# michaelriedl/2048-ppo-agent

Measured on AMD Instinct MI355X. Metric: env-steps/sec at N parallel boards (full PPO loop: rollout with policy in the loop + GAE + update), higher is better.
Workload: dtype u8 boards / bf16 policy; 1 GPU; 65536 parallel boards per GPU, Transformer policy bf16 (3.96 M params), full PPO iteration (BASELINE.json configs[2]; configs[3] when n_gpus=8); boards_per_gpu=65536, global_boards=65536, train_batch=2048, update_epochs=5, max_samples_per_epoch=300000, max_samples_per_epoch_is=global (each rank draws its 1/N share), as the reference's single subset, max_samples_per_epoch_per_rank=300000, rollout_mode=episodes (reference lock-step semantics), rng_mode=partitionable, parallelism=env-shard x1 + 1 grad all-reduce/minibatch

## Files before the change

2048-ppo-agent_amd/csrc/g2048_linear.hip:

```cpp
#include <hip/hip_runtime.h>
#include <stdint.h>

#include "../../include/g2048.h"
#include "g2048_colsum_final.h"
#include "g2048_host.h"
#include "g2048_mfma.h"

namespace {

using namespace g2048_mfma;
using namespace g2048_host;

enum { EPI_NONE = 0, EPI_RELU_DROPOUT = 1, EPI_MASK_COLSUM = 2 };
struct Epi {
    float inv_keep;
    uint32_t thr16, s0, s1;
    const uint64_t *seed_state;
    int64_t row_elems;
    uint2 *bits;
    float *partial;
    int N;
    uint32_t hi_term;
};

constexpr int TOK = 128, NS = 128, KC = 128, THREADS = 256;
constexpr int CHUNK_BYTES = NS * KC * 2;
constexpr int NBUF = 2;

__device__ __forceinline__ void dma_chunk(char *dst, const __bf16 *w_slice, int64_t ldw, int kc, int w, int lane) {
    const char *base = reinterpret_cast<const char *>(w_slice) + (size_t)kc * KC * 2;
    for (int t = 0; t < NS / 16; ++t) {
        const int row = 4 * (4 * t + w) + (lane >> 4);
        const int q = (lane & 15) ^ (row & 15);
        const char *g = base + (size_t)row * ldw * 2 + q * 16;
        __builtin_amdgcn_global_load_lds((const __attribute__((address_space(1))) void *)g,
                                         (__attribute__((address_space(3))) void *)(dst + (4 * t + w) * 1024), 16, 0, 0);
    }
}

template <bool HAS_BIAS, int EPI>
__device__ __forceinline__ void store_tile(f32x16 acc[4], const float *__restrict__ bias, __bf16 *yrow, int n0, int h, bool valid,
                                           const Epi &E, int64_t tok, uint2 *bits_slot, uint2 bits_in, float *colacc) {
    uint32_t obits[2] = {0u, 0u};
    const uint32_t pair0 = (uint32_t)(((uint64_t)tok * (uint64_t)E.row_elems + (uint64_t)(n0 + 4 * h)) >> 1);
    for (int j = 0; j < 4; ++j) {
        if (HAS_BIAS)
            for (int g = 0; g < 4; ++g) {
                const float4 bv = *reinterpret_cast<const float4 *>(bias + n0 + 32 * j + 8 * g + 4 * h);
                acc[j][4 * g + 0] += bv.x; acc[j][4 * g + 1] += bv.y; acc[j][4 * g + 2] += bv.z; acc[j][4 * g + 3] += bv.w;
            }
        if (EPI == EPI_RELU_DROPOUT) {
            for (int i = 0; i < 16; i += 2) {
                float a = fmaxf(acc[j][i], 0.f), b = fmaxf(acc[j][i + 1], 0.f);
                if (E.thr16) {
                    uint32_t x = (pair0 + (uint32_t)(16 * j + ((i & 3) >> 1) + 4 * (i >> 2))) * HASH_MUL + E.hi_term;
                    G2048_HASH_FIN(x);
                    a = (x & 0xFFFFu) >= E.thr16 ? a * E.inv_keep : 0.f;
                    b = (x >> 16) >= E.thr16 ? b * E.inv_keep : 0.f;
                }
                acc[j][i] = a; acc[j][i + 1] = b;
            }
        }
        if (EPI == EPI_MASK_COLSUM) {
            const uint32_t w = j < 2 ? bits_in.x : bits_in.y;
            for (int i = 0; i < 16; ++i) acc[j][i] = ((w >> (16 * (j & 1) + i)) & 1u) ? acc[j][i] * E.inv_keep : 0.f;
        }
        for (int m = 0; m < 2; ++m) {
            uint32_t ax = pack2(acc[j][8 * m + 0], acc[j][8 * m + 1]), ay = pack2(acc[j][8 * m + 2], acc[j][8 * m + 3]);
            uint32_t bx = pack2(acc[j][8 * m + 4], acc[j][8 * m + 5]), by = pack2(acc[j][8 * m + 6], acc[j][8 * m + 7]);
            if (EPI == EPI_RELU_DROPOUT) {
                const uint32_t pk[4] = {ax, ay, bx, by};
                for (int q = 0; q < 4; ++q) {
                    const uint32_t nz = ((pk[q] & 0x7FFFu) ? 1u : 0u) | ((pk[q] & 0x7FFF0000u) ? 2u : 0u);
                    obits[j >> 1] |= nz << (16 * (j & 1) + 8 * m + 2 * q);
                }
            }
            const auto sx = __builtin_amdgcn_permlane32_swap(ax, bx, false, false);
            const auto sy = __builtin_amdgcn_permlane32_swap(ay, by, false, false);
            uint32_t o[4] = {sx[0], sy[0], sx[1], sy[1]};
            if (EPI == EPI_MASK_COLSUM) {
                for (int q = 0; q < 4; ++q) {
                    if (!valid) o[q] = 0u;
                    colacc[8 * (2 * j + m) + 2 * q] += __uint_as_float(o[q] << 16);
                    colacc[8 * (2 * j + m) + 2 * q + 1] += __uint_as_float(o[q] & 0xFFFF0000u);
                }
            }
            if (valid) *reinterpret_cast<uint4 *>(yrow + 32 * j + 16 * m) = make_uint4(o[0], o[1], o[2], o[3]);
        }
    }
    if (EPI == EPI_RELU_DROPOUT && bits_slot) *bits_slot = make_uint2(obits[0], obits[1]);
}

template <bool HAS_BIAS>
__global__ void __launch_bounds__(THREADS, 2)
k_linear(const __bf16 *__restrict__ x, int64_t ldx, const __bf16 *__restrict__ wgt, int64_t ldw, const float *__restrict__ bias,
         __bf16 *__restrict__ y, int64_t ldy, int64_t T, int K) {
    extern __shared__ __attribute__((aligned(16))) char smem[];
    const int tid = threadIdx.x, lane = tid & 63, w = tid >> 6, r = lane & 31, h = lane >> 5;
    const int64_t tok0 = (int64_t)blockIdx.x * TOK + 32 * w;
    const int n0 = blockIdx.y * NS;
    const __bf16 *w_slice = wgt + (size_t)n0 * ldw;
    const int n_chunks = K / KC;

    int64_t tok = tok0 + r;
    const bool valid = tok < T;
    if (!valid) tok = T - 1;
    const uint4 *xrow = reinterpret_cast<const uint4 *>(x + tok * ldx) + h;

    uint4 bq[8];
    for (int ks = 0; ks < 8; ++ks) bq[ks] = xrow[2 * ks];
    dma_chunk(smem, w_slice, ldw, 0, w, lane);
    if (n_chunks > 1) dma_chunk(smem + CHUNK_BYTES, w_slice, ldw, 1, w, lane);

    f32x16 acc[4];
    for (int j = 0; j < 4; ++j)
        for (int i = 0; i < 16; ++i) acc[j][i] = 0.f;

    int aoff[8];
    for (int ks = 0; ks < 8; ++ks) aoff[ks] = r * 256 + (((2 * ks + h) ^ (r & 15)) * 16);

    for (int c = 0; c < n_chunks; ++c) {
        if (c + 1 < n_chunks) asm volatile("s_waitcnt vmcnt(8)" ::: "memory");
        else asm volatile("s_waitcnt vmcnt(0)" ::: "memory");
        __syncthreads();
        const char *tile = smem + (c % NBUF) * CHUNK_BYTES;
        bf16x8 b[8];
        for (int ks = 0; ks < 8; ++ks) b[ks] = *reinterpret_cast<const bf16x8 *>(&bq[ks]);
        if (c + 1 < n_chunks)
            for (int ks = 0; ks < 8; ++ks) bq[ks] = xrow[2 * (8 * (c + 1) + ks)];
        for (int ks = 0; ks < 8; ++ks)
            for (int j = 0; j < 4; ++j) {
                const bf16x8 a = *reinterpret_cast<const bf16x8 *>(tile + aoff[ks] + j * 32 * 256);
                acc[j] = __builtin_amdgcn_mfma_f32_32x32x16_bf16(a, b[ks], acc[j], 0, 0, 0);
            }
        __syncthreads();
        if (c + NBUF < n_chunks) dma_chunk(smem + (c % NBUF) * CHUNK_BYTES, w_slice, ldw, c + NBUF, w, lane);
    }
    store_tile<HAS_BIAS, EPI_NONE>(acc, bias, y + (tok0 + r) * ldy + n0 + 8 * h, n0, h, valid, Epi{}, 0, nullptr, make_uint2(0u, 0u), nullptr);
}


constexpr int TOKW = 64;
template <int K, int NF>
struct XTileDma {
    static constexpr int CPR = K / 8, RPI = 64 / CPR, N_INST = TOKW / RPI;
    static constexpr int NVAR = 16 / RPI / NF > 0 ? 16 / RPI / NF : 1;
    static_assert(N_INST % NF == 0, "every wave issues the same number of fetch instructions");
    uint32_t voff[NVAR];
    int sub, p;
    __device__ __forceinline__ void init(int64_t ldx, int lane, int f) {
        sub = lane / CPR, p = lane % CPR;
        for (int v = 0; v < NVAR; ++v)
            voff[v] = (uint32_t)(sub * ldx * 2) + 16u * (uint32_t)(p ^ ((RPI * (NF * v + f) + sub) & 15));
    }
    __device__ __forceinline__ void full(char *dst, const __bf16 *x, int64_t ldx, int64_t tok0, int f) const {
        const char *base = reinterpret_cast<const char *>(x + tok0 * ldx);
#pragma unroll
        for (int j = 0; j < N_INST / NF; ++j) {
            const int n = NF * j + f;
            dma_async16(base + (int64_t)n * RPI * ldx * 2, voff[j % NVAR], dst + n * 1024);
        }
    }
    __device__ __forceinline__ void clamped(char *dst, const __bf16 *x, int64_t ldx, int64_t tok0, int64_t T, int f) const {
        for (int j = 0; j < N_INST / NF; ++j) {
            const int n = NF * j + f;
            const int row = n * RPI + sub;
            int64_t tok = tok0 + row;
            if (tok >= T) tok = T - 1;
            dma_async<16>(reinterpret_cast<const char *>(x + tok * ldx) + (p ^ (row & 15)) * 16, dst + n * 1024);
        }
    }
};

#ifdef G2048_WS_STAMPS
constexpr int WS_PHASES = 8;
__device__ unsigned long long g_ws_stamps[2][WS_PHASES];
struct WsStampSite {
    __device__ __forceinline__ static bool on(int lane, int w) { return lane == 0 && w < 2 && blockIdx.y == 0 && blockIdx.x % 16 == 0; }
    __device__ __forceinline__ static unsigned long long *table(int w) { return g_ws_stamps[w == 0 ? 0 : 1]; }
};
#define WS_STAMP(k) stamps.mark(k)
#else
#define WS_STAMP(k)
#endif

template <bool HAS_BIAS, int EPI, int KS, int WAVES>
__global__ void __launch_bounds__(64 * WAVES, 1)
k_linear_ws(const __bf16 *__restrict__ x, int64_t ldx, const __bf16 *__restrict__ wgt, int64_t ldw, const float *__restrict__ bias,
            __bf16 *__restrict__ y, int64_t ldy, int64_t T, Epi E) {
    constexpr int THREADS = 64 * WAVES, NSW = 32 * WAVES;
    constexpr int CPR_Y = NSW / 8;
    constexpr int K = 16 * KS;
    extern __shared__ __attribute__((aligned(16))) char smem[];
    const int tid = threadIdx.x, lane = tid & 63, r = lane & 31, h = lane >> 5;
    const int w = __builtin_amdgcn_readfirstlane(tid >> 6);
    const int n0 = blockIdx.y * NSW;
    constexpr int row_bytes = K * 2, xbytes = TOKW * row_bytes, sbytes = TOKW * 2 * NSW;

    bf16x8 wf[KS];
    {
        const __bf16 *wrow = wgt + (size_t)(n0 + 32 * w + r) * ldw + 8 * h;
#pragma unroll
        for (int ks = 0; ks < KS; ++ks) wf[ks] = *reinterpret_cast<const bf16x8 *>(wrow + 16 * ks);
    }
    constexpr int NB = 2;
    char *const stage = smem + NB * xbytes;
    float *const bias_l = reinterpret_cast<float *>(smem + NB * xbytes + sbytes);
    uint32_t *const bits_l = reinterpret_cast<uint32_t *>(smem + NB * xbytes + sbytes + NSW * 4);
    for (int i = tid; i < NSW; i += THREADS) bias_l[i] = HAS_BIAS ? bias[n0 + i] : 0.f;
    if (EPI == EPI_RELU_DROPOUT) {
        mix_seed_state(E.seed_state, E.s0, E.s1);
        E.hi_term = E.s0 ^ (E.s1 * HASH_MUL_HI);
    }
    const int slices = gridDim.y;
    float colacc[EPI == EPI_MASK_COLSUM ? 16 : 1];
    for (int q = 0; q < (EPI == EPI_MASK_COLSUM ? 16 : 1); ++q) colacc[q] = 0.f;
    const int64_t n_tiles64 = (T + TOKW - 1) / TOKW;
    auto bits_ptr = [&](int64_t tile) -> uint32_t * {
        return reinterpret_cast<uint32_t *>(E.bits) + (tile * slices + blockIdx.y) * THREADS;
    };
    XTileDma<K, WAVES> dma;
    dma.init(ldx, lane, w);
    auto fetch = [&](int64_t tile, int buf) {
        if ((tile + 1) * TOKW <= T) dma.full(smem + buf * xbytes, x, ldx, tile * TOKW, w);
        else dma.clamped(smem + buf * xbytes, x, ldx, tile * TOKW, T, w);
        if (EPI == EPI_MASK_COLSUM) {
            const uint32_t *g = bits_ptr(tile) + lane;
            dma_async<4>(g + 64 * w, bits_l + buf * THREADS + 64 * w);
        }
    };
    if ((int64_t)blockIdx.x < n_tiles64) fetch(blockIdx.x, 0);
    asm volatile("s_waitcnt vmcnt(0)" ::: "memory");
#ifdef G2048_WS_STAMPS
    Stamps<WS_PHASES, WsStampSite> stamps;
    stamps.start();
#endif
    int buf = 0;
    for (int64_t tile = blockIdx.x; tile < n_tiles64; tile += gridDim.x, buf ^= 1) {
        const int64_t tok0 = tile * TOKW;
        const char *const xb = smem + buf * xbytes;
        lds_barrier_asm();
        WS_STAMP(1);
        if (tile + gridDim.x < n_tiles64) fetch(tile + gridDim.x, buf ^ 1);
        WS_STAMP(2);
        const uint32_t bits_in = EPI == EPI_MASK_COLSUM ? bits_l[buf * THREADS + tid] : 0u;
        f32x16 acc[2];
        for (int g = 0; g < 4; ++g) {
            const float4 bv = *reinterpret_cast<const float4 *>(bias_l + 32 * w + 8 * g + 4 * h);
            for (int b = 0; b < 2; ++b) {
                acc[b][4 * g + 0] = bv.x; acc[b][4 * g + 1] = bv.y; acc[b][4 * g + 2] = bv.z; acc[b][4 * g + 3] = bv.w;
            }
        }
        const int nw = n0 + 32 * w;
        uint32_t obits = 0u;
        auto keep_pair = [&](int pi, uint32_t pair0) -> uint32_t {
            const int i = 2 * pi;
            uint32_t xh = (pair0 + (uint32_t)(((i & 3) >> 1) + 4 * (i >> 2))) * HASH_MUL + E.hi_term;
            G2048_HASH_FIN(xh);
            return ((xh & 0xFFFFu) >= E.thr16 ? 1u : 0u) | ((xh >> 16) >= E.thr16 ? 2u : 0u);
        };
        auto drop_pair = [&](int b, int pi, uint32_t keep) {
            const int i = 2 * pi;
            const float a = fmaxf(acc[b][i], 0.f), c = fmaxf(acc[b][i + 1], 0.f);
            acc[b][i] = (keep & 1u) ? a * E.inv_keep : 0.f;
            acc[b][i + 1] = (keep & 2u) ? c * E.inv_keep : 0.f;
        };
        auto finish_g = [&](int b, int g, bool valid) {
            if (EPI == EPI_MASK_COLSUM) {
                const uint32_t wbits = bits_in >> (16 * b + 4 * g);
#pragma unroll
                for (int j = 0; j < 4; ++j) acc[b][4 * g + j] = ((wbits >> j) & 1u) ? acc[b][4 * g + j] * E.inv_keep : 0.f;
            }
            const uint32_t lo = pack2(acc[b][4 * g + 0], acc[b][4 * g + 1]), hi = pack2(acc[b][4 * g + 2], acc[b][4 * g + 3]);
            if (EPI == EPI_RELU_DROPOUT) {
                const uint32_t nz = ((lo & 0x7FFFu) ? 1u : 0u) | ((lo & 0x7FFF0000u) ? 2u : 0u) | ((hi & 0x7FFFu) ? 4u : 0u) |
                                    ((hi & 0x7FFF0000u) ? 8u : 0u);
                obits |= nz << (16 * b + 4 * g);
            }
            if (EPI == EPI_MASK_COLSUM) {
                colacc[4 * g + 0] += valid ? __uint_as_float(lo << 16) : 0.f;
                colacc[4 * g + 1] += valid ? __uint_as_float(lo & 0xFFFF0000u) : 0.f;
                colacc[4 * g + 2] += valid ? __uint_as_float(hi << 16) : 0.f;
                colacc[4 * g + 3] += valid ? __uint_as_float(hi & 0xFFFF0000u) : 0.f;
            }
            const int trow = 32 * b + r, c = 4 * w + g;
            *reinterpret_cast<uint2 *>(stage + trow * (2 * NSW) + ((c ^ (trow & (CPR_Y - 1))) * 16) + 8 * h) = make_uint2(lo, hi);
        };
        const bool valid0 = tok0 + r < T, valid1 = tok0 + 32 + r < T;
        uint32_t pair0[2];
        for (int b = 0; b < 2; ++b)
            pair0[b] = (uint32_t)(((uint64_t)((b ? valid1 : valid0) ? tok0 + 32 * b + r : T - 1) * (uint64_t)E.row_elems + (uint64_t)(nw + 4 * h)) >> 1);
        {
            constexpr int PRE = 8, N = 2 * KS;
            bf16x8 q[PRE];
            auto frag = [&](int s) {
                const int b = s / KS, ks = s % KS;
                return *reinterpret_cast<const bf16x8 *>(xb + (32 * b + r) * row_bytes + (((2 * ks + h) ^ (r & 15)) * 16));
            };
#pragma unroll
            for (int s = 0; s < PRE; ++s) q[s] = frag(s);
#pragma unroll
            for (int s = 0; s < N; ++s) {
                __builtin_amdgcn_sched_barrier(0);
                const int b = s / KS, ks = s % KS;
                acc[b] = __builtin_amdgcn_mfma_f32_32x32x16_bf16(wf[ks], q[s % PRE], acc[b], 0, 0, 0);
                if (s + PRE < N) q[s % PRE] = frag(s + PRE);
                constexpr int SPG = KS / 4;
                const int g = ks / SPG, t = ks % SPG;
                if (b == 1) {
                    if (EPI == EPI_RELU_DROPOUT) {
                        if (SPG >= 4) {
                            if (t == 0) drop_pair(0, 2 * g, keep_pair(2 * g, pair0[0]));
                            if (t == 2) drop_pair(0, 2 * g + 1, keep_pair(2 * g + 1, pair0[0]));
                        } else if (t == 0) {
                            drop_pair(0, 2 * g, keep_pair(2 * g, pair0[0]));
                            drop_pair(0, 2 * g + 1, keep_pair(2 * g + 1, pair0[0]));
                        }
                    }
                    if (t == SPG - 1) finish_g(0, g, valid0);
                }
            }
            __builtin_amdgcn_sched_barrier(0);
        }
        WS_STAMP(3);
#pragma unroll
        for (int g = 0; g < 4; ++g) {
            if (EPI == EPI_RELU_DROPOUT) {
                drop_pair(1, 2 * g, keep_pair(2 * g, pair0[1]));
                drop_pair(1, 2 * g + 1, keep_pair(2 * g + 1, pair0[1]));
            }
            finish_g(1, g, valid1);
        }
        if (EPI == EPI_RELU_DROPOUT && E.bits) bits_ptr(tile)[tid] = obits;
        WS_STAMP(5);
        asm volatile("s_waitcnt vmcnt(0)" ::: "memory");
        WS_STAMP(0);
        lds_barrier_asm();
        WS_STAMP(6);
        {
            constexpr int PIECES = TOKW * CPR_Y, STORERS = THREADS, ROUNDS = PIECES / STORERS;
            static_assert(PIECES % STORERS == 0, "every lane moves the same number of 16-byte pieces");
            const int e0 = tid;
            uint4 v[ROUNDS];
#pragma unroll
            for (int i = 0; i < ROUNDS; ++i) {
                const int e = e0 + STORERS * i;
                v[i] = *reinterpret_cast<const uint4 *>(stage + (e / CPR_Y) * (2 * NSW) + (e % CPR_Y) * 16);
            }
#pragma unroll
            for (int i = 0; i < ROUNDS; ++i) {
                const int e = e0 + STORERS * i;
                const int trow = e / CPR_Y, p = e % CPR_Y, c = p ^ (trow & (CPR_Y - 1));
                if (tok0 + trow < T) *reinterpret_cast<uint4 *>(y + (tok0 + trow) * ldy + n0 + 8 * c) = v[i];
            }
        }
        WS_STAMP(7);
    }
#ifdef G2048_WS_STAMPS
    stamps.flush(lane, w);
#endif
    if (EPI == EPI_MASK_COLSUM) {
        for (int q = 0; q < 16; ++q) {
            float v = colacc[q];
            for (int m = 16; m >= 1; m >>= 1) v += __shfl_xor(v, m);
            if (r == 0) E.partial[(int64_t)blockIdx.x * E.N + n0 + 32 * w + rowof(q, h)] = v;
        }
    }
}

}

namespace {

inline int ws_waves(int N) { return N % 256 == 0 ? 8 : 4; }
inline int64_t ws_groups(int64_t T, int N) {
    const int waves = ws_waves(N);
    const int64_t n_tiles = (T + TOKW - 1) / TOKW;
    int64_t groups = 256 / (N / (32 * waves));
    if (groups < 1) groups = 1;
    if (groups >= 8) groups -= groups % 8;
    return groups > n_tiles ? n_tiles : groups;
}

inline bool operands_ok(const void *x, int64_t ldx, const void *weight, int64_t ldw, const void *y, int64_t ldy, int64_t T, int K,
                        int N, const void *bias) {
    return x && weight && y && T > 0 && K >= KC && K % KC == 0 && N >= NS && N % NS == 0 && ldx >= K && ldw >= K && ldy >= N &&
           !(ldx & 7) && !(ldw & 7) && !(ldy & 7) && aligned16(x, weight, y, bias);
}

template <bool HAS_BIAS, int EPI, int KS, int WAVES>
int launch_ws(const __bf16 *x, int64_t ldx, const __bf16 *w, int64_t ldw, const float *bias, __bf16 *y, int64_t ldy, int64_t T, int N,
              const Epi &E, int64_t groups, hipStream_t stream) {
    const void *fn = reinterpret_cast<const void *>(k_linear_ws<HAS_BIAS, EPI, KS, WAVES>);
    const int lds = 2 * TOKW * 16 * KS * 2 + TOKW * 2 * 32 * WAVES + 32 * WAVES * 4 + 2 * 64 * WAVES * 4;
    if (const int rc = allow_dynamic_lds(fn, lds)) return rc;
    hipLaunchKernelGGL((k_linear_ws<HAS_BIAS, EPI, KS, WAVES>), dim3((unsigned)groups, (unsigned)(N / (32 * WAVES))), dim3(64 * WAVES), lds,
                       stream, x, ldx, w, ldw, bias, y, ldy, T, E);
    return launch_status();
}
template <bool HAS_BIAS, int EPI>
int launch_stationary(const __bf16 *x, int64_t ldx, const __bf16 *w, int64_t ldw, const float *bias, __bf16 *y, int64_t ldy, int64_t T,
                      int K, int N, const Epi &E, int *groups_out, hipStream_t stream) {
    if (K != 256 && K != 128) return G2048_EINVAL;
    const int64_t groups = ws_groups(T, N);
    if (groups_out) *groups_out = (int)groups;
    const bool wide = ws_waves(N) == 8;
    if (K == 256)
        return wide ? launch_ws<HAS_BIAS, EPI, 16, 8>(x, ldx, w, ldw, bias, y, ldy, T, N, E, groups, stream)
                    : launch_ws<HAS_BIAS, EPI, 16, 4>(x, ldx, w, ldw, bias, y, ldy, T, N, E, groups, stream);
    return wide ? launch_ws<HAS_BIAS, EPI, 8, 8>(x, ldx, w, ldw, bias, y, ldy, T, N, E, groups, stream)
                : launch_ws<HAS_BIAS, EPI, 8, 4>(x, ldx, w, ldw, bias, y, ldy, T, N, E, groups, stream);
}

}

extern "C" int g2048_linear_bf16(const void *x, int64_t ldx, const void *weight, int64_t ldw, const float *bias, void *y,
                                 int64_t ldy, int64_t T, int K, int N, void *stream) {
    if (!operands_ok(x, ldx, weight, ldw, y, ldy, T, K, N, bias)) return G2048_EINVAL;
    const __bf16 *xp = (const __bf16 *)x, *wp = (const __bf16 *)weight;
    __bf16 *yp = (__bf16 *)y;
    if (K <= NBUF * KC)
        return bias ? launch_stationary<true, EPI_NONE>(xp, ldx, wp, ldw, bias, yp, ldy, T, K, N, Epi{}, nullptr, (hipStream_t)stream)
                    : launch_stationary<false, EPI_NONE>(xp, ldx, wp, ldw, bias, yp, ldy, T, K, N, Epi{}, nullptr, (hipStream_t)stream);
    const void *fn = bias ? reinterpret_cast<const void *>(k_linear<true>) : reinterpret_cast<const void *>(k_linear<false>);
    if (const int rc = allow_dynamic_lds(fn, NBUF * CHUNK_BYTES)) return rc;
    const dim3 grid((unsigned)((T + TOK - 1) / TOK), (unsigned)(N / NS));
    if (bias)
        hipLaunchKernelGGL(k_linear<true>, grid, dim3(THREADS), NBUF * CHUNK_BYTES, (hipStream_t)stream, xp, ldx, wp, ldw, bias, yp, ldy, T, K);
    else
        hipLaunchKernelGGL(k_linear<false>, grid, dim3(THREADS), NBUF * CHUNK_BYTES, (hipStream_t)stream, xp, ldx, wp, ldw, bias, yp, ldy, T,
                           K);
    return launch_status();
}

extern "C" int64_t g2048_ffn_mask_bytes(int64_t T, int N) {
    return (T <= 0 || N < NS || N % NS) ? 0 : ((T + TOK - 1) / TOK) * (N / NS) * THREADS * (int64_t)sizeof(uint2);
}

extern "C" int g2048_linear_relu_dropout_bf16(const void *x, int64_t ldx, const void *weight, int64_t ldw, const float *bias, void *y,
                                              int64_t ldy, int64_t T, int K, int N, float p_drop, uint64_t seed,
                                              const uint64_t *seed_state, void *mask_bits, void *stream) {
    if (!operands_ok(x, ldx, weight, ldw, y, ldy, T, K, N, bias) || !bias || K > NBUF * KC || !(p_drop >= 0.f && p_drop < 1.f))
        return G2048_EINVAL;
    Epi E{};
    E.inv_keep = 1.0f / (1.0f - p_drop);
    E.thr16 = (uint32_t)(p_drop * 65536.0f + 0.5f);
    E.s0 = (uint32_t)seed; E.s1 = (uint32_t)(seed >> 32);
    E.seed_state = p_drop > 0.f ? seed_state : nullptr;
    E.row_elems = N;
    E.bits = (uint2 *)mask_bits;
    if ((uintptr_t)mask_bits & 7) return G2048_EINVAL;
    return launch_stationary<true, EPI_RELU_DROPOUT>((const __bf16 *)x, ldx, (const __bf16 *)weight, ldw, bias, (__bf16 *)y, ldy, T, K, N,
                                                     E, nullptr, (hipStream_t)stream);
}

extern "C" int64_t g2048_linear_mask_bwd_workspace_floats(int64_t T, int N) {
    return (T <= 0 || N < NS || N % NS) ? 0 : (int64_t)512 * N;
}

extern "C" int64_t g2048_linear_mask_bwd_partial_rows(int64_t T, int N) {
    if (T <= 0 || N < NS || N % NS) return 0;
    return ws_groups(T, N);
}

extern "C" int g2048_linear_mask_bwd_bf16(const void *dy, int64_t lddy, const void *weight_t, int64_t ldw, const void *mask_bits,
                                          void *dz, int64_t lddz, float *dbias, float *workspace, int64_t T, int K, int N,
                                          float p_drop, void *stream) {
    if (!operands_ok(dy, lddy, weight_t, ldw, dz, lddz, T, K, N, nullptr) || K > NBUF * KC || !mask_bits ||
        ((uintptr_t)mask_bits & 7) || !workspace || !aligned16(workspace) || !(p_drop >= 0.f && p_drop < 1.f))
        return G2048_EINVAL;
    Epi E{};
    E.inv_keep = 1.0f / (1.0f - p_drop);
    E.bits = (uint2 *)const_cast<void *>(mask_bits);
    E.partial = workspace;
    E.N = N;
    int groups = 0;
    const int rc = launch_stationary<false, EPI_MASK_COLSUM>((const __bf16 *)dy, lddy, (const __bf16 *)weight_t, ldw, nullptr, (__bf16 *)dz,
                                                             lddz, T, K, N, E, &groups, (hipStream_t)stream);
    if (rc || !dbias) return rc;
    hipLaunchKernelGGL(k_colsum_final, dim3((unsigned)((N + CF_COLS - 1) / CF_COLS)), dim3(CF_COLS * CF_SLICES), 0, (hipStream_t)stream,
                       workspace, groups, N, dbias);
    return launch_status();
}

#ifdef G2048_WS_STAMPS
extern "C" int g2048_debug_ws_stamps(unsigned long long *out , int reset) {
    if (hipMemcpyFromSymbol(out, HIP_SYMBOL(g_ws_stamps), sizeof(g_ws_stamps)) != hipSuccess) return -1;
    if (reset) {
        static const unsigned long long zero[2][WS_PHASES] = {};
        if (hipMemcpyToSymbol(HIP_SYMBOL(g_ws_stamps), zero, sizeof(zero)) != hipSuccess) return -1;
    }
    return 0;
}
#endif
```

include/g2048.h:

```cpp
#ifndef G2048_H
#define G2048_H

#include <stdint.h>

#ifdef __cplusplus
extern "C" {
#endif

#define G2048_ABI_VERSION 4
#define G2048_EINVAL (-1)
#define G2048_RNG_LEGACY 0
#define G2048_RNG_PARTITIONABLE 1
#define G2048_POLICY_DRUL 0
#define G2048_POLICY_RANDOM 1
#define G2048_MAX_FUSED_STEPS 128

int g2048_abi_version(void);


int g2048_split(uint32_t key0, uint32_t key1, uint32_t *out_keys, int64_t n, int rng_mode, void *stream);

int g2048_chain_keys(uint32_t *key , uint32_t *subs , int64_t n, int rng_mode);


int g2048_init(const uint32_t *keys, uint8_t *boards, uint8_t *masks, uint8_t *done, int64_t B,
               int rng_mode, void *stream);

int g2048_step(uint8_t *boards, uint8_t *masks, uint8_t *done, const int32_t *actions,
               const uint32_t *keys, float *rewards, int64_t B, int rng_mode, void *stream);

int g2048_observe(const uint8_t *boards, uint8_t *obs, int64_t B, void *stream);


int g2048_act_drul(const uint8_t *masks, int32_t *actions, int64_t B, void *stream);
int g2048_act_random(const uint32_t *keys, const uint8_t *masks, int32_t *actions, float *log_probs,
                     int64_t B, int rng_mode, void *stream);
int g2048_act_logits(const uint32_t *keys, const float *logits, const uint8_t *masks, int use_mask,
                     int sample, int32_t *actions, float *log_probs, int64_t B, int rng_mode, void *stream);


int g2048_reset_fused(uint32_t sub0, uint32_t sub1, uint8_t *boards, uint8_t *masks, uint8_t *done,
                      int32_t *ep_len, int64_t B, int64_t B_total, int64_t env0, int rng_mode, void *stream);

int g2048_rollout_fused(const uint32_t *step_subs , int n_steps, int64_t t0, uint8_t *boards,
                        uint8_t *masks, uint8_t *done, int32_t *ep_len, uint8_t *tr_boards,
                        uint8_t *tr_meta, float *tr_rewards, float *tr_logp, int64_t B, int64_t B_total,
                        int64_t env0, int policy, int fill_frozen, int rng_mode, uint32_t *live_count,
                        void *stream);

int g2048_policy_step(uint32_t act_sub0, uint32_t act_sub1, uint32_t step_sub0, uint32_t step_sub1,
                      const float *logits, const float *values, int use_mask, int sample, int64_t t,
                      uint8_t *boards, uint8_t *masks, uint8_t *done, int32_t *ep_len, uint8_t *tr_boards,
                      uint8_t *tr_meta, float *tr_rewards, float *tr_logp, float *tr_values, int64_t B,
                      int64_t B_total, int64_t env0, int fill_frozen, int rng_mode, uint32_t *live_count,
                      void *stream);

int g2048_policy_step_autoreset(uint32_t act_sub0, uint32_t act_sub1, uint32_t step_sub0, uint32_t step_sub1,
                                const float *logits, const float *values, int use_mask, int sample, int64_t t,
                                uint8_t *boards, uint8_t *masks, int32_t *ep_len, uint8_t *tr_boards, uint8_t *tr_meta,
                                float *tr_rewards, float *tr_logp, float *tr_values, int64_t B, int64_t B_total,
                                int64_t env0, int rng_mode, void *stream);
int g2048_reset_key(uint32_t step_sub0, uint32_t step_sub1, uint32_t *out );


int g2048_gae_tb(const float *tr_rewards, const float *tr_values, const int32_t *ep_len, float *tr_adv,
                 float *tr_ret, int64_t T, int64_t B, double gamma, double lam, void *stream);

int g2048_gae_tb_boot(const float *tr_rewards, const float *tr_values, const uint8_t *tr_meta, const float *last_values,
                      float *tr_adv, float *tr_ret, int64_t T, int64_t B, double gamma, double lam, void *stream);

int g2048_gae_flat(const float *rewards, const float *values, const uint8_t *terms, float *adv, float *ret,
                   int64_t N, double gamma, double lam, void *stream);

int g2048_compact(const uint8_t *tr_boards, const uint8_t *tr_meta, const float *tr_rewards, const float *tr_logp,
                  const float *tr_values, const float *tr_adv, const float *tr_ret, const int32_t *ep_len,
                  const int64_t *offsets, uint8_t *out_boards, uint8_t *out_actions, uint8_t *out_masks, float *out_rewards,
                  float *out_logp, float *out_values, float *out_adv, float *out_ret, uint8_t *out_terms, int64_t T,
                  int64_t B, void *stream);


int64_t g2048_policy_encoder_workspace_bytes(int64_t B);
int g2048_policy_encoder(const uint8_t *boards, const float *embed_table, const float *cls_token,
                         const void *weights_bf16, const float *params_f32, int n_layers, float *features,
                         int64_t B, void *workspace, void *stream);

int g2048_policy_encoder_mean(const uint8_t *boards, const float *embed_table, const float *cls_token,
                              const void *weights_bf16, const float *params_f32, int n_layers, float *features,
                              int64_t B, void *stream);

#define G2048_F32SPLIT_BIAS 0
#define G2048_F32SPLIT_BIAS_RELU 1
#define G2048_F32SPLIT_ADD_LN 2
#define G2048_F32SPLIT_ADD 3

int g2048_f32split_pack(const float *w, int N, int K, float scale, void *packed, void *stream);

int g2048_f32split_gemm(const float *x, int64_t ldx, const void *w_packed, const float *bias, float *y, int64_t ldy,
                        const float *resid, const float *gamma, const float *beta, float *h, int64_t T, int K, int N,
                        int epilogue, float sx, float sw, float eps, void *stream);

int g2048_attn_fwd_f32(const float *qkv, float *o, int64_t B, int H, float scale, void *stream);

int g2048_embed_ln_f32(const uint8_t *boards, const float *table, const float *cls, const float *gamma, const float *beta, float eps,
                       float *x0, float *h, int64_t B, void *stream);


int g2048_lookahead_expand(const uint8_t *boards, int64_t B, uint8_t *after, float *reward, int32_t *nchild, void *stream);

int g2048_lookahead_children(const uint8_t *after, const int32_t *nchild, const int32_t *offset, int64_t B, int64_t N,
                             uint8_t *children, uint8_t *terminal, void *stream);

int g2048_lookahead_reduce(const float *reward, const int32_t *nchild, const int32_t *offset, const float *values,
                           const uint8_t *terminal, double gamma, int64_t B, int64_t N, float *q, void *stream);


int g2048_lookahead_dedup(const uint8_t *after, const int32_t *nchild, const int32_t *group_start, int64_t G, int64_t P, int32_t *rep,
                          int32_t *nuniq, void *stream);

int g2048_lookahead_backup(const float *reward, const int32_t *nchild, const int32_t *rep, const float *e, int64_t N1, float *v1,
                           void *stream);


int g2048_sym_canon(const uint8_t *boards, const uint8_t *actions, const uint8_t *masks, int64_t B, uint8_t *out_boards,
                    uint8_t *out_actions, uint8_t *out_masks, uint8_t *frame, void *stream);

int g2048_sym_logits(const float *logits, const uint8_t *frame, int64_t B, float *out, void *stream);


int g2048_sym_views(const uint8_t *boards, int64_t B, uint8_t *views, void *stream);

int g2048_sym_fold(const float *logits, const float *values, int64_t B, float *out_logits, float *out_values, void *stream);


int g2048_mc_playout(const uint32_t *step_subs , int n_steps, int64_t t0, const uint8_t *roots, int64_t B, int R,
                     int64_t lane0, int64_t n_total, int policy, double gamma, uint8_t *lane_boards, uint8_t *lane_masks,
                     uint8_t *lane_done, float *lane_ret, float *lane_disc, int rng_mode, uint32_t *live_count, void *stream);

int g2048_mc_reduce(const float *lane_ret, const float *lane_disc, const uint8_t *lane_done, const float *leaf_values, int64_t B,
                    int R, float *q, void *stream);


int g2048_ntuple_values(const uint8_t *boards, int64_t n, const int32_t *weights, const uint8_t *tuple_cells , int m, int L,
                        int frac_bits, float *values, void *stream);

int g2048_ntuple_scores(const uint8_t *boards, int64_t B, const int32_t *weights, const uint8_t *tuple_cells , int m, int L,
                        int frac_bits, float *scores, float *values, void *stream);

int g2048_ntuple_td_accumulate(const uint8_t *prev_after, const uint8_t *flag, const float *target, int64_t B,
                               const int32_t *weights, const uint8_t *tuple_cells , int m, int L, int frac_bits, double alpha,
                               int64_t *acc, int32_t *cnt, float *td_error, void *stream);

int g2048_ntuple_td_apply(const uint8_t *prev_after, const uint8_t *flag, int64_t B, const uint8_t *tuple_cells , int m, int L,
                          int32_t *weights, int64_t *acc, int32_t *cnt, void *stream);

int g2048_ntuple_link(const uint8_t *tr_boards_row, const uint8_t *tr_meta_row, int64_t B, uint8_t *prev_after, uint8_t *flag,
                      void *stream);


int64_t g2048_ntuple_expectimax_workspace_floats(int64_t B, int plies);

int g2048_ntuple_expectimax(const uint8_t *boards, int64_t B, const int32_t *weights, const uint8_t *tuple_cells , int m,
                            int L, int frac_bits, int plies, double gamma, float *workspace, float *scores, float *values,
                            void *stream);


int g2048_ntuple_tc_accumulate(const uint8_t *prev_after, const uint8_t *flag, const float *target, int64_t B,
                               const int32_t *weights, const uint8_t *tuple_cells , int m, int L, int frac_bits, double alpha,
                               int64_t *acc, int64_t *abs_acc, int32_t *cnt, float *td_error, void *stream);

int g2048_ntuple_tc_apply(const uint8_t *prev_after, const uint8_t *flag, int64_t B, const uint8_t *tuple_cells , int m, int L,
                          int32_t *weights, int64_t *acc, int64_t *abs_acc, int32_t *cnt, int32_t *coh_e, int32_t *coh_a,
                          void *stream);

int g2048_ntuple_staged_values(const uint8_t *boards, int64_t n, const int32_t *weights, const uint8_t *tuple_cells , int m,
                               int L, const uint8_t *stage_tiles , int n_stages, int frac_bits, float *values, void *stream);
int g2048_ntuple_staged_scores(const uint8_t *boards, int64_t B, const int32_t *weights, const uint8_t *tuple_cells , int m,
                               int L, const uint8_t *stage_tiles , int n_stages, int frac_bits, float *scores, float *values,
                               void *stream);
int g2048_ntuple_staged_expectimax(const uint8_t *boards, int64_t B, const int32_t *weights, const uint8_t *tuple_cells ,
                                   int m, int L, const uint8_t *stage_tiles , int n_stages, int frac_bits, int plies,
                                   double gamma, float *workspace, float *scores, float *values, void *stream);
int g2048_ntuple_staged_td_accumulate(const uint8_t *prev_after, const uint8_t *flag, const float *target, int64_t B,
                                      const int32_t *weights, const uint8_t *tuple_cells , int m, int L,
                                      const uint8_t *stage_tiles , int n_stages, int frac_bits, double alpha, int64_t *acc,
                                      int32_t *cnt, float *td_error, void *stream);
int g2048_ntuple_staged_td_apply(const uint8_t *prev_after, const uint8_t *flag, int64_t B, const uint8_t *tuple_cells , int m,
                                 int L, const uint8_t *stage_tiles , int n_stages, int32_t *weights, int64_t *acc,
                                 int32_t *cnt, void *stream);
int g2048_ntuple_staged_tc_accumulate(const uint8_t *prev_after, const uint8_t *flag, const float *target, int64_t B,
                                      const int32_t *weights, const uint8_t *tuple_cells , int m, int L,
                                      const uint8_t *stage_tiles , int n_stages, int frac_bits, double alpha, int64_t *acc,
                                      int64_t *abs_acc, int32_t *cnt, float *td_error, void *stream);
int g2048_ntuple_staged_tc_apply(const uint8_t *prev_after, const uint8_t *flag, int64_t B, const uint8_t *tuple_cells , int m,
                                 int L, const uint8_t *stage_tiles , int n_stages, int32_t *weights, int64_t *acc,
                                 int64_t *abs_acc, int32_t *cnt, int32_t *coh_e, int32_t *coh_a, void *stream);


int g2048_attn_fwd(const void *q, const void *k, const void *v, void *o, float *lse, int64_t B, int H, int Sq,
                   int64_t q_sb, int64_t q_ss, int64_t k_sb, int64_t k_ss, int64_t v_sb, int64_t v_ss, float scale,
                   float p_drop, uint64_t seed, const uint64_t *seed_state, void *stream);
int g2048_attn_bwd(const void *q, const void *k, const void *v, const void *dout, const float *lse, void *dq, void *dk,
                   void *dv, int64_t B, int H, int Sq, int64_t q_sb, int64_t q_ss, int64_t k_sb, int64_t k_ss,
                   int64_t v_sb, int64_t v_ss, float scale, float p_drop, uint64_t seed, const uint64_t *seed_state,
                   void *stream);


int g2048_add_ln_fwd(const float *x, int64_t x_row_stride, const void *a, const float *gamma, const float *beta,
                     float *x_new, void *h, float *mean, float *rstd, int64_t T, float eps, float p_drop,
                     uint64_t seed, const uint64_t *seed_state, void *stream);
int64_t g2048_add_ln_bwd_workspace_floats(int64_t T);
int g2048_add_ln_bwd(const float *x_norm, int64_t x_row_stride, const float *g_x, const void *g_h, const float *mean,
                     const float *rstd, const float *gamma, float *dx, void *da, float *dparams, float *workspace,
                     int64_t T, float p_drop, uint64_t seed, const uint64_t *seed_state, int g_x_period, void *stream);


int g2048_linear_add_ln_fwd(const void *u, int64_t ldu, const void *w_packed, const float *bias, int K, const float *x,
                            int64_t x_row_stride, const float *gamma, const float *beta, float *x_new, void *h, float *mean,
                            float *rstd, int64_t T, float eps, float p_drop, uint64_t seed, const uint64_t *seed_state, void *stream);
int64_t g2048_linear_add_ln_bwd_partial_rows(int64_t T);
int g2048_linear_add_ln_bwd(const void *dy, int64_t lddy, const void *wt_packed, int64_t wt_tile_stride, int K, const float *x_norm,
                            int64_t x_row_stride, const float *g_x, int g_x_period, const void *g_h_extra, int extra_period,
                            const float *mean, const float *rstd, const float *gamma, float *dx, void *da, float *partial, int64_t T,
                            float p_drop, uint64_t seed, const uint64_t *seed_state, void *stream);


int g2048_mlp_embed_fwd(const uint8_t *boards, const void *wt, const float *bias, void *y, void *onehot, int64_t M, void *stream);

#define G2048_GEMM_MAX_JOBS 8
typedef struct {
    const void *x[2]; int64_t ldx[2];
    const void *w[2]; int64_t ldw[2];
    int32_t k[2];
    const float *bias;
    const void *act; int64_t ldact;
    void *y; int64_t ldy;
    int32_t N, relu;
} g2048_gemm_job;
int g2048_gemm_jobs(const g2048_gemm_job *jobs, int n_jobs, int64_t M, void *stream);

int g2048_mlp_out_fwd(const void *h2, const void *w3, float *logits, float *values, int64_t M, void *stream);
int64_t g2048_mlp_out_bwd_partial_rows(int64_t M);
int g2048_mlp_out_bwd(const float *dlogits, const float *dvalues, const void *h2, const void *w3, void *dh2, float *partial, int64_t M,
                      void *stream);


#define G2048_COLSUM_MAX_GROUPS 512
int64_t g2048_colsum_workspace_floats(int64_t T, int N);
int64_t g2048_colsum_partial_rows(int64_t T, int N);
int g2048_colsum(const void *x, int is_bf16, int64_t row_stride, int64_t T, int N, float *workspace, float *out,
                 void *stream);


#define G2048_PPO_LOSS_MAX_BATCH 1048576
int g2048_ppo_loss(const void *logits, int logits_bf16, const void *values, int values_bf16, const uint8_t *actions,
                   const uint8_t *mask_bits, const float *old_logp, const float *adv, const float *ret, int64_t M,
                   float clip_eps, float c_value, float c_entropy, float *new_logp, float *sums, void *dlogits,
                   void *dvalues, const float *grad_scale, double *running, void *stream);


int64_t g2048_distill_loss_workspace_floats(int64_t M);

int g2048_distill_loss(const void *logits, int logits_bf16, const void *values, int values_bf16, const uint8_t *mask_bits,
                       const float *teacher_q, const float *value_target, int64_t M, float tau, float c_value, float c_entropy,
                       float *new_logp, float *sums, void *dlogits, void *dvalues, const float *grad_scale, double *running,
                       float *workspace, void *stream);

int g2048_distill_gather(const int64_t *idx, int64_t M, int64_t N, const uint8_t *boards, const uint8_t *masks, const float *teacher_q,
                         const float *value_target, uint8_t *o_boards, uint8_t *o_masks, float *o_q, float *o_vt, void *stream);


int g2048_relu_dropout_fwd(const void *x, void *y, int64_t T, int F, float p_drop, uint64_t seed,
                           const uint64_t *seed_state, void *stream);
int64_t g2048_relu_dropout_bwd_workspace_floats(int64_t T, int F);
int g2048_relu_dropout_bwd(const void *dy, const void *y, void *dx, float *dbias, float *workspace, int64_t T, int F,
                           float p_drop, void *stream);


int g2048_dweight_bf16(const void *dy, int64_t lddy, const void *x, int64_t ldx, void *parts, float *colsum, int64_t T, int N,
                       int K, int slices, int block_rows, void *stream);

#define G2048_DWG_MAX_JOBS 16
typedef struct {
    const void *dy; const void *x; void *parts; float *colsum;
    int64_t lddy, ldx, T;
    int32_t N, K, slices, parts_f32;
} g2048_dwg_job;
int g2048_dweight_jobs(const g2048_dwg_job *jobs, int n_jobs, void *stream);
int g2048_dweight_jobs_tiled(const g2048_dwg_job *jobs, int n_jobs, int big_cells, void *stream);
int g2048_dweight_jobs_plan(const g2048_dwg_job *jobs, int n_jobs, int big_cells, int cus, int32_t *n_big);


int g2048_linear_bf16(const void *x, int64_t ldx, const void *weight, int64_t ldw, const float *bias, void *y, int64_t ldy,
                      int64_t T, int K, int N, void *stream);

int64_t g2048_ffn_mask_bytes(int64_t T, int N);
int g2048_linear_relu_dropout_bf16(const void *x, int64_t ldx, const void *weight, int64_t ldw, const float *bias, void *y,
                                   int64_t ldy, int64_t T, int K, int N, float p_drop, uint64_t seed,
                                   const uint64_t *seed_state, void *mask_bits, void *stream);
int64_t g2048_linear_mask_bwd_workspace_floats(int64_t T, int N);
int64_t g2048_linear_mask_bwd_partial_rows(int64_t T, int N);
int g2048_linear_mask_bwd_bf16(const void *dy, int64_t lddy, const void *weight_t, int64_t ldw, const void *mask_bits, void *dz,
                               int64_t lddz, float *dbias, float *workspace, int64_t T, int K, int N, float p_drop,
                               void *stream);


int g2048_embed_fwd(const uint8_t *boards, const float *wt, int w_ld, const float *pe, const float *cls, float *x0, int64_t M,
                    float p_drop, uint64_t seed, const uint64_t *seed_state, void *stream);
int g2048_embed_ln_fwd(const uint8_t *boards, const float *wt, int w_ld, const float *pe, const float *cls, float *x0, int64_t M,
                       float p_drop, uint64_t seed, const uint64_t *seed_state, const float *gamma, const float *beta, float eps,
                       void *h, float *mean, float *rstd, void *stream);
int64_t g2048_embed_bwd_workspace_floats(int64_t M);
int g2048_embed_bwd(const uint8_t *boards, const float *dx0, float *dwt_dcls, float *workspace, int64_t M, float p_drop,
                    uint64_t seed, const uint64_t *seed_state, void *stream);



#define G2048_REDUCE_MAX_JOBS 64
typedef struct {
    const void *src; float *dst; int64_t part_stride; int32_t n, parts, src_bf16, transpose_rows;
} g2048_reduce_job;
int g2048_reduce_jobs(const g2048_reduce_job *jobs, int n_jobs, void *stream);


#define G2048_OPT_CHUNK 2048
#define G2048_OPT_MAX_GROUPS 4
typedef struct {
    float *param; int64_t offset; int32_t n; int32_t group;
    void *shadow;
    void *shadow_t;
    void *shadow_p;
    void *shadow_tp;
    int32_t e0;
    int32_t rows, cols;
    int32_t reserved;
} g2048_opt_chunk;
typedef struct { double lr, beta1, beta2, eps, weight_decay; } g2048_opt_group;
int64_t g2048_opt_workspace_floats(int n_chunks);
int g2048_opt_step(const g2048_opt_chunk *chunks, int n_chunks, const float *grads, float *exp_avg, float *exp_avg_sq,
                   const g2048_opt_group *groups, int n_groups, float max_grad_norm, float *steps, int n_steps, float *scale,
                   int32_t *growth_tracker, float growth, float backoff, int growth_interval, float *workspace,
                   float *info, void *stream);

typedef struct { double lr, beta1, beta2, beta3, eps, weight_decay;
                 int32_t bias_correction, adapt, trust_clip, reserved; } g2048_lamb_group;
int64_t g2048_lamb_workspace_floats(int n_chunks);
int g2048_lamb_step(const g2048_opt_chunk *chunks, int n_chunks, const float *grads, float *exp_avg, float *exp_avg_sq,
                    const g2048_lamb_group *groups, int n_groups, float max_grad_norm, float lamb_max_grad_norm,
                    float *steps, int n_steps, float *scale, int32_t *growth_tracker, float growth, float backoff,
                    int growth_interval, float *workspace, float *info, void *stream);


typedef struct {
    const void *wo, *w1, *w2;
    const void *a1, *a2, *a3;
    const void *c1, *c2, *c3;
    const float *bo, *b1, *b2, *ab1, *ab2, *cb1, *cb2;
    const float *ln_g, *ln_b;
} g2048_tail_weights;
typedef struct {
    const void *woT, *w1T, *w2T;
    const void *a1T, *a2T, *a3;
    const void *c1T, *c2T, *c3;
    const float *ln_g;
} g2048_tail_weights_t;
#define G2048_TAIL_MASK_TILES 96
typedef struct {
    float *x_mid, *mean, *rstd;
    void *masks;
    void *oT, *h2T, *uT, *featsT;
    void *a1T, *a2T, *c1T, *c2T;
    int64_t ld;
} g2048_tail_saved;
typedef struct {
    void *daoT, *dzT, *df2T;
    void *da1T, *da2T, *dlT;
    void *dc1T, *dc2T, *dvT;
    float *ln_partial;
} g2048_tail_grads;
int g2048_cls_tail_fwd(const void *o, const float *x_cls, int64_t x_row_stride, const g2048_tail_weights *W,
                       const g2048_tail_saved *S, float *logits, float *values, int64_t M, float eps, float p_drop, uint64_t seed,
                       const uint64_t *seed_state, void *stream);
int g2048_cls_tail_bwd(const float *dlogits, const float *dvalues, const g2048_tail_weights_t *WT, const g2048_tail_saved *S,
                       const g2048_tail_grads *G, void *d_o, float *dx_cls, int64_t M, float p_drop, uint64_t seed,
                       const uint64_t *seed_state, void *stream);

#define G2048_DW_MAX_JOBS 16
typedef struct { const void *dyT; const void *xT; float *dw; float *db; int32_t N, K; } g2048_dw_job;
int g2048_dweight_t(const g2048_dw_job *jobs, int n_jobs, int64_t ld, int64_t m, int slices, void *stream);

int g2048_gather_minibatch(const int64_t *idx, int64_t M, int64_t N, const uint8_t *boards, const uint8_t *actions,
                           const uint8_t *masks, const float *logp, const float *adv, const float *ret, uint8_t *o_boards,
                           uint8_t *o_actions, uint8_t *o_masks, float *o_logp, float *o_adv, float *o_ret, void *stream);

#ifdef __cplusplus
}
#endif
#endif
```

Before: 3.997 million env-steps/sec.

## Fit two 4-wave linear workgroups per CU and default non-colsum paths to 4 waves

Bias moves from LDS into per-lane registers and the colsum mask bits are loaded straight into a register instead of through an LDS DMA. This shrinks the kernel's LDS footprint so two 4-wave workgroups can share a CU, and the launch bounds now ask for that. The wave-count choice changes too: non-colsum epilogues on N divisible by 256 now default to the 4-wave variant, with an environment override, hoping the doubled residency overlaps DMA and MFMA better. In exchange it costs extra registers under a tighter register budget and adds occupancy query APIs.

```diff
diff --git a/2048-ppo-agent_amd/csrc/g2048_linear.hip b/2048-ppo-agent_amd/csrc/g2048_linear.hip
--- a/2048-ppo-agent_amd/csrc/g2048_linear.hip
+++ b/2048-ppo-agent_amd/csrc/g2048_linear.hip
@@ -1,5 +1,6 @@
 #include <hip/hip_runtime.h>
 #include <stdint.h>
+#include <stdlib.h>
 
 #include "../../include/g2048.h"
 #include "g2048_colsum_final.h"
@@ -141,6 +142,7 @@
 
 
 constexpr int TOKW = 64;
+constexpr int ws_lds_bytes(int KS, int WAVES) { return 2 * TOKW * 16 * KS * 2 + TOKW * 2 * 32 * WAVES; }
 template <int K, int NF>
 struct XTileDma {
     static constexpr int CPR = K / 8, RPI = 64 / CPR, N_INST = TOKW / RPI;
@@ -185,7 +187,7 @@
 #endif
 
 template <bool HAS_BIAS, int EPI, int KS, int WAVES>
-__global__ void __launch_bounds__(64 * WAVES, 1)
+__global__ void __launch_bounds__(64 * WAVES, WAVES == 4 ? 2 : 1)
 k_linear_ws(const __bf16 *__restrict__ x, int64_t ldx, const __bf16 *__restrict__ wgt, int64_t ldw, const float *__restrict__ bias,
             __bf16 *__restrict__ y, int64_t ldy, int64_t T, Epi E) {
     constexpr int THREADS = 64 * WAVES, NSW = 32 * WAVES;
@@ -205,9 +207,13 @@
     }
     constexpr int NB = 2;
     char *const stage = smem + NB * xbytes;
-    float *const bias_l = reinterpret_cast<float *>(smem + NB * xbytes + sbytes);
-    uint32_t *const bits_l = reinterpret_cast<uint32_t *>(smem + NB * xbytes + sbytes + NSW * 4);
-    for (int i = tid; i < NSW; i += THREADS) bias_l[i] = HAS_BIAS ? bias[n0 + i] : 0.f;
+    static_assert(NB * xbytes + sbytes == ws_lds_bytes(KS, WAVES), "the kernel's LDS map and the launch's byte count");
+    float bias_r[HAS_BIAS ? 16 : 1];
+    if (HAS_BIAS)
+        for (int g = 0; g < 4; ++g) {
+            const float4 bv = *reinterpret_cast<const float4 *>(bias + n0 + 32 * w + 8 * g + 4 * h);
+            bias_r[4 * g + 0] = bv.x; bias_r[4 * g + 1] = bv.y; bias_r[4 * g + 2] = bv.z; bias_r[4 * g + 3] = bv.w;
+        }
     if (EPI == EPI_RELU_DROPOUT) {
         mix_seed_state(E.seed_state, E.s0, E.s1);
         E.hi_term = E.s0 ^ (E.s1 * HASH_MUL_HI);
@@ -221,16 +227,18 @@
     };
     XTileDma<K, WAVES> dma;
     dma.init(ldx, lane, w);
+    uint32_t bits_next = 0u;
     auto fetch = [&](int64_t tile, int buf) {
         if ((tile + 1) * TOKW <= T) dma.full(smem + buf * xbytes, x, ldx, tile * TOKW, w);
         else dma.clamped(smem + buf * xbytes, x, ldx, tile * TOKW, T, w);
-        if (EPI == EPI_MASK_COLSUM) {
-            const uint32_t *g = bits_ptr(tile) + lane;
-            dma_async<4>(g + 64 * w, bits_l + buf * THREADS + 64 * w);
-        }
+        if (EPI == EPI_MASK_COLSUM) bits_next = bits_ptr(tile)[tid];
+    };
+    auto ws_landed = [&]() {
+        if (EPI == EPI_MASK_COLSUM) asm volatile("s_waitcnt vmcnt(0)" : "+v"(bits_next)::"memory");
+        else asm volatile("s_waitcnt vmcnt(0)" ::: "memory");
     };
     if ((int64_t)blockIdx.x < n_tiles64) fetch(blockIdx.x, 0);
-    asm volatile("s_waitcnt vmcnt(0)" ::: "memory");
+    ws_landed();
 #ifdef G2048_WS_STAMPS
     Stamps<WS_PHASES, WsStampSite> stamps;
     stamps.start();
@@ -241,16 +249,12 @@
         const char *const xb = smem + buf * xbytes;
         lds_barrier_asm();
         WS_STAMP(1);
+        const uint32_t bits_in = bits_next;
         if (tile + gridDim.x < n_tiles64) fetch(tile + gridDim.x, buf ^ 1);
         WS_STAMP(2);
-        const uint32_t bits_in = EPI == EPI_MASK_COLSUM ? bits_l[buf * THREADS + tid] : 0u;
         f32x16 acc[2];
-        for (int g = 0; g < 4; ++g) {
-            const float4 bv = *reinterpret_cast<const float4 *>(bias_l + 32 * w + 8 * g + 4 * h);
-            for (int b = 0; b < 2; ++b) {
-                acc[b][4 * g + 0] = bv.x; acc[b][4 * g + 1] = bv.y; acc[b][4 * g + 2] = bv.z; acc[b][4 * g + 3] = bv.w;
-            }
-        }
+        for (int b = 0; b < 2; ++b)
+            for (int i = 0; i < 16; ++i) acc[b][i] = HAS_BIAS ? bias_r[i] : 0.f;
         const int nw = n0 + 32 * w;
         uint32_t obits = 0u;
         auto keep_pair = [&](int pi, uint32_t pair0) -> uint32_t {
@@ -333,7 +337,7 @@
         }
         if (EPI == EPI_RELU_DROPOUT && E.bits) bits_ptr(tile)[tid] = obits;
         WS_STAMP(5);
-        asm volatile("s_waitcnt vmcnt(0)" ::: "memory");
+        ws_landed();
         WS_STAMP(0);
         lds_barrier_asm();
         WS_STAMP(6);
@@ -372,15 +376,24 @@
 
 namespace {
 
-inline int ws_waves(int N) { return N % 256 == 0 ? 8 : 4; }
+inline int ws_plan_waves(int N) { return N % 256 == 0 ? 8 : 4; }
 inline int64_t ws_groups(int64_t T, int N) {
-    const int waves = ws_waves(N);
+    const int waves = ws_plan_waves(N);
     const int64_t n_tiles = (T + TOKW - 1) / TOKW;
     int64_t groups = 256 / (N / (32 * waves));
     if (groups < 1) groups = 1;
     if (groups >= 8) groups -= groups % 8;
     return groups > n_tiles ? n_tiles : groups;
 }
+template <bool HAS_BIAS, int EPI>
+constexpr bool ws_pair_default() { return EPI != EPI_MASK_COLSUM; }
+template <bool HAS_BIAS, int EPI>
+inline int ws_waves(int N) {
+    if (N % 256) return 4;
+    const char *e = getenv("G2048_WS_WIDE");
+    if (e && (e[0] == '0' || e[0] == '1') && !e[1]) return e[0] == '1' ? 8 : 4;
+    return ws_pair_default<HAS_BIAS, EPI>() ? 4 : 8;
+}
 
 inline bool operands_ok(const void *x, int64_t ldx, const void *weight, int64_t ldw, const void *y, int64_t ldy, int64_t T, int K,
                         int N, const void *bias) {
@@ -392,7 +405,8 @@
 int launch_ws(const __bf16 *x, int64_t ldx, const __bf16 *w, int64_t ldw, const float *bias, __bf16 *y, int64_t ldy, int64_t T, int N,
               const Epi &E, int64_t groups, hipStream_t stream) {
     const void *fn = reinterpret_cast<const void *>(k_linear_ws<HAS_BIAS, EPI, KS, WAVES>);
-    const int lds = 2 * TOKW * 16 * KS * 2 + TOKW * 2 * 32 * WAVES + 32 * WAVES * 4 + 2 * 64 * WAVES * 4;
+    constexpr int lds = ws_lds_bytes(KS, WAVES);
+    static_assert(WAVES != 4 || 2 * lds <= 160 * 1024, "two 4-wave workgroups share a CU's LDS");
     if (const int rc = allow_dynamic_lds(fn, lds)) return rc;
     hipLaunchKernelGGL((k_linear_ws<HAS_BIAS, EPI, KS, WAVES>), dim3((unsigned)groups, (unsigned)(N / (32 * WAVES))), dim3(64 * WAVES), lds,
                        stream, x, ldx, w, ldw, bias, y, ldy, T, E);
@@ -404,7 +418,7 @@
     if (K != 256 && K != 128) return G2048_EINVAL;
     const int64_t groups = ws_groups(T, N);
     if (groups_out) *groups_out = (int)groups;
-    const bool wide = ws_waves(N) == 8;
+    const bool wide = ws_waves<HAS_BIAS, EPI>(N) == 8;
     if (K == 256)
         return wide ? launch_ws<HAS_BIAS, EPI, 16, 8>(x, ldx, w, ldw, bias, y, ldy, T, N, E, groups, stream)
                     : launch_ws<HAS_BIAS, EPI, 16, 4>(x, ldx, w, ldw, bias, y, ldy, T, N, E, groups, stream);
@@ -431,6 +445,37 @@
         hipLaunchKernelGGL(k_linear<false>, grid, dim3(THREADS), NBUF * CHUNK_BYTES, (hipStream_t)stream, xp, ldx, wp, ldw, bias, yp, ldy, T,
                            K);
     return launch_status();
+}
+
+extern "C" int64_t g2048_linear_ws_lds_bytes(int K, int waves) {
+    return ((K != 128 && K != 256) || (waves != 4 && waves != 8)) ? 0 : ws_lds_bytes(K / 16, waves);
+}
+
+namespace {
+
+template <bool HAS_BIAS, int EPI, int KS, int WAVES>
+int ws_resident() {
+    int n = 0;
+    if (hipOccupancyMaxActiveBlocksPerMultiprocessor(&n, k_linear_ws<HAS_BIAS, EPI, KS, WAVES>, 64 * WAVES, ws_lds_bytes(KS, WAVES)) != hipSuccess) {
+        (void)hipGetLastError();
+        return -1;
+    }
+    return n;
+}
+template <int KS, int WAVES>
+int ws_resident_min() {
+    const int n[4] = {ws_resident<true, EPI_NONE, KS, WAVES>(), ws_resident<false, EPI_NONE, KS, WAVES>(),
+                      ws_resident<true, EPI_RELU_DROPOUT, KS, WAVES>(), ws_resident<false, EPI_MASK_COLSUM, KS, WAVES>()};
+    int m = n[0];
+    for (int i = 1; i < 4; ++i) m = n[i] < m ? n[i] : m;
+    return m;
+}
+}
+
+extern "C" int g2048_linear_ws_workgroups_per_cu(int K, int waves) {
+    if ((K != 128 && K != 256) || (waves != 4 && waves != 8)) return G2048_EINVAL;
+    if (K == 256) return waves == 4 ? ws_resident_min<16, 4>() : ws_resident_min<16, 8>();
+    return waves == 4 ? ws_resident_min<8, 4>() : ws_resident_min<8, 8>();
 }
 
 extern "C" int64_t g2048_ffn_mask_bytes(int64_t T, int N) {
diff --git a/include/g2048.h b/include/g2048.h
--- a/include/g2048.h
+++ b/include/g2048.h
@@ -292,6 +292,8 @@
 
 int g2048_linear_bf16(const void *x, int64_t ldx, const void *weight, int64_t ldw, const float *bias, void *y, int64_t ldy,
                       int64_t T, int K, int N, void *stream);
+int64_t g2048_linear_ws_lds_bytes(int K, int waves);
+int g2048_linear_ws_workgroups_per_cu(int K, int waves);
 
 int64_t g2048_ffn_mask_bytes(int64_t T, int N);
 int g2048_linear_relu_dropout_bf16(const void *x, int64_t ldx, const void *weight, int64_t ldw, const float *bias, void *y,
```

New measurement: 4.013 million env-steps/sec (median of 6 runs). About the same (+0.4%).
